# EternityJune25/ComoRAG

Hardware: NVIDIA H100
Metric: queries/sec (higher is better)
Workload: dtype bf16

## Files before the change

comorag_b200/_native.py:

```python
from __future__ import annotations

import ctypes as C
import threading
from pathlib import Path

LIB_PATH = Path(__file__).resolve().parent / "lib" / "libcomorag_b200.so"

CRAG_OK = 0


class NativeError(RuntimeError):
    """A libcomorag_b200 entry point returned a non-zero status."""


_c_i64p = C.POINTER(C.c_int64)
_c_f32p = C.POINTER(C.c_float)

SIGNATURES = {
    "crag_version": (C.c_int, []),
    "crag_last_error": (C.c_char_p, []),
    "crag_sm_count": (C.c_int, []),
    "crag_vmem_reserve": (C.c_int, [C.c_size_t, C.POINTER(C.c_uint64), C.POINTER(C.c_size_t)]),
    "crag_vmem_grow": (C.c_int, [C.c_uint64, C.c_size_t, C.c_size_t]),
    "crag_vmem_release": (C.c_int, [C.c_uint64, C.c_size_t, C.c_size_t]),
    "crag_search_workspace_bytes": (C.c_size_t, [C.c_int, C.c_int]),
    "crag_search_topk": (C.c_int, [C.c_void_p, C.c_int64, C.c_int, C.c_int64, C.c_int64, C.c_void_p, C.c_int,
                                   C.c_int, C.c_void_p, C.c_void_p, C.c_void_p, C.c_void_p, C.c_size_t,
                                   C.c_void_p]),
    "crag_gemm_bf16": (C.c_int, [C.c_void_p, C.c_int64, C.c_void_p, C.c_int64, C.c_void_p, C.c_void_p, C.c_int64,
                                 C.c_void_p, C.c_int64, C.c_int, C.c_int, C.c_int, C.c_int, C.c_void_p]),
    "crag_pool_normalize": (C.c_int, [C.c_void_p, C.c_void_p, C.c_int, C.c_int, C.c_int, C.c_void_p, C.c_void_p,
                                      C.c_int64, C.c_void_p]),
    "crag_encoder_workspace_bytes": (C.c_size_t, None),
    "crag_encoder_forward": (C.c_int, None),
    "crag_encoder_classify": (C.c_int, None),
    "crag_attention_varlen": (C.c_int, [C.c_void_p, C.c_void_p, C.c_int, C.c_int, C.c_int, C.c_int, C.c_void_p,
                                        C.c_void_p]),
    "crag_attention_varlen_tc": (C.c_int, [C.c_void_p, C.c_void_p, C.c_int, C.c_int, C.c_int, C.c_int, C.c_int,
                                           C.c_void_p, C.c_void_p]),
    "crag_layernorm": (C.c_int, [C.c_void_p, C.c_int, C.c_int, C.c_void_p, C.c_void_p, C.c_float, C.c_void_p,
                                 C.c_void_p]),
    "crag_search_topk_after": (C.c_int, [C.c_void_p, C.c_int64, C.c_int, C.c_int64, C.c_int64, C.c_void_p, C.c_int,
                                         C.c_int, C.c_void_p, C.c_void_p, C.c_void_p, C.c_void_p, C.c_void_p,
                                         C.c_void_p, C.c_size_t, C.c_void_p]),
    "crag_search_scan": (C.c_int, [C.c_void_p, C.c_int64, C.c_int, C.c_int64, C.c_void_p, C.c_int, C.c_int, C.c_void_p,
                                   C.c_size_t, C.c_void_p]),
    "crag_search_finalize": (C.c_int, [C.c_void_p, C.c_size_t, C.c_int64, C.c_int, C.c_int, C.c_int64, C.c_void_p,
                                       C.c_void_p, C.c_void_p, C.c_void_p]),
    "crag_merge_topk_packed": (C.c_int, [C.c_void_p, C.c_int64, C.c_int, C.c_int, C.c_int, C.c_void_p, C.c_void_p,
                                         C.c_void_p, C.c_void_p]),
    "crag_ivf_workspace_bytes": (C.c_size_t, [C.c_int, C.c_int64, C.c_int]),
    "crag_ivf_search": (C.c_int, [C.c_void_p, C.c_int64, C.c_int, C.c_int64, C.c_void_p, C.c_void_p, C.c_int, C.c_int64,
                                  C.c_void_p, C.c_void_p, C.c_int, C.c_void_p, C.c_void_p, C.c_int, C.c_int, C.c_void_p,
                                  C.c_void_p, C.c_void_p, C.c_void_p, C.c_size_t, C.c_void_p]),
    "crag_exchange_buffer_bytes": (C.c_size_t, [C.c_int]),
    "crag_search_finalize_exchange": (C.c_int, [C.c_void_p, C.c_size_t, C.c_int64, C.c_int, C.c_int, C.c_int64, C.c_void_p,
                                                C.c_int, C.c_int, C.c_void_p, C.c_void_p, C.c_void_p, C.c_void_p,
                                                C.c_void_p, C.c_void_p]),
    "crag_ivf_assign": (C.c_int, [C.c_void_p, C.c_int64, C.c_int, C.c_int64, C.c_void_p, C.c_int, C.c_void_p, C.c_void_p,
                                  C.c_void_p, C.c_size_t, C.c_void_p]),
    "crag_search_scores": (C.c_int, [C.c_void_p, C.c_int64, C.c_int, C.c_int64, C.c_void_p, C.c_int, C.c_void_p, C.c_int64,
                                     C.c_void_p, C.c_void_p, C.c_size_t, C.c_void_p]),
    "crag_rank_workspace_bytes": (C.c_size_t, [C.c_int64]),
# ... 65 lines not shown
```

comorag_b200/csrc/gemm.cu:

```cuda
#include <cstdlib>

#include "common.cuh"
#include "gemm.cuh"
#include "ptx.cuh"

namespace crag {

constexpr int kGemmBM = 128;
constexpr int kGemmBN = 128;
constexpr int kGemmBK = 64;
constexpr int kGemmConsumerWarps = 8;
constexpr int kGemmThreads = 32 * kGemmConsumerWarps + 32;
constexpr int kGemmStages = 3;

struct GemmLayout {
  static constexpr int kABytes = kGemmBM * kGemmBK * 2;
  static constexpr int kBBytes = kGemmBN * kGemmBK * 2;
  static constexpr int kStageBytes = kABytes + kBBytes;
  static constexpr size_t smem_bytes() { return 1024 + size_t(kGemmStages) * kStageBytes + 2 * kGemmStages * 8; }
};

__device__ __forceinline__ float gelu_erf(float x) {
  const float z = x * 0.70710678118654752f;
  const float az = fabsf(z);
  float t;
  asm("rcp.approx.ftz.f32 %0, %1;" : "=f"(t) : "f"(fmaf(0.3275911f, az, 1.0f)));
  float p = fmaf(1.061405429f, t, -1.453152027f);
  p = fmaf(p, t, 1.421413741f);
  p = fmaf(p, t, -0.284496736f);
  p = fmaf(p, t, 0.254829592f);
  p *= t;
  float e;
  asm("ex2.approx.ftz.f32 %0, %1;" : "=f"(e) : "f"(az * az * -1.4426950408889634f));
  const float erf_abs = fmaf(-p, e, 1.0f);
  const float half_x = 0.5f * x;
  return fmaf(half_x, copysignf(erf_abs, z), half_x);
}

__device__ __forceinline__ uint32_t pack_bf16x2(float a, float b) {
  __nv_bfloat162 v = __floats2bfloat162_rn(a, b);
  return *reinterpret_cast<uint32_t*>(&v);
}

template <int EPI>
__global__ void __launch_bounds__(kGemmThreads, 2)
gemm_bf16_kernel(const __grid_constant__ CUtensorMap tm_a, const __grid_constant__ CUtensorMap tm_b, int M, int N,
                 int K, const float* __restrict__ bias, const __nv_bfloat16* __restrict__ residual, int64_t ldr,
                 __nv_bfloat16* __restrict__ out, int64_t ldo) {
  using L = GemmLayout;
  constexpr int STAGES = kGemmStages;
  extern __shared__ uint8_t smem_raw[];
  uint8_t* smem = reinterpret_cast<uint8_t*>((reinterpret_cast<uintptr_t>(smem_raw) + 1023) & ~uintptr_t(1023));
  uint64_t* bar_full = reinterpret_cast<uint64_t*>(smem + STAGES * L::kStageBytes);
  uint64_t* bar_empty = bar_full + STAGES;

  const int warp = threadIdx.x >> 5;
  const int lane = threadIdx.x & 31;
  int n_blk = blockIdx.x, m_blk = blockIdx.y;
  if constexpr (EPI == GEMM_EPI_SCORES_F32) {
    const int m_blocks = (M + kGemmBM - 1) / kGemmBM;
    m_blk = int(blockIdx.x % unsigned(m_blocks));
    n_blk = int(blockIdx.x / unsigned(m_blocks));
  }
  const int num_kb = (K + kGemmBK - 1) / kGemmBK;

  if (threadIdx.x == 0) {
    for (int s = 0; s < STAGES; ++s) {
      mbar_init(&bar_full[s], 1);
      mbar_init(&bar_empty[s], kGemmConsumerWarps);
    }
    fence_mbar_init();
  }
  __syncthreads();

  if (warp == kGemmConsumerWarps) {
    if (lane == 0) {
      tma_prefetch_desc(&tm_a);
      tma_prefetch_desc(&tm_b);
      const uint64_t pol_w = policy_evict_last();
      int stage = 0;
      uint32_t phase = 0;
      for (int kb = 0; kb < num_kb; ++kb) {
        mbar_wait(&bar_empty[stage], phase ^ 1);
        uint8_t* sa = smem + stage * L::kStageBytes;
        mbar_arrive_expect_tx(&bar_full[stage], L::kStageBytes);
        tma_load_2d(&tm_a, &bar_full[stage], sa, kb * kGemmBK, m_blk * kGemmBM);
        tma_load_2d_hint(&tm_b, &bar_full[stage], sa + L::kABytes, kb * kGemmBK, n_blk * kGemmBN, pol_w);
        if (++stage == STAGES) { stage = 0; phase ^= 1; }
      }
    }
    return;
  }

  const int wg = warp >> 2;
  float acc[kGemmBN / 2];
#pragma unroll
  for (int i = 0; i < kGemmBN / 2; ++i) acc[i] = 0.f;
  int stage = 0, prev = 0;
  uint32_t phase = 0;
  for (int kb = 0; kb < num_kb; ++kb) {
    mbar_wait(&bar_full[stage], phase);
    const uint32_t a_addr = smem_u32(smem + stage * L::kStageBytes) + wg * 64 * 128;
    const uint32_t b_addr = smem_u32(smem + stage * L::kStageBytes + L::kABytes);
    wgmma_fence();
#pragma unroll
    for (int ks = 0; ks < kGemmBK / 16; ++ks)
      wgmma_m64n128k16_ss(acc, wgmma_desc_sw128(a_addr + ks * 32), wgmma_desc_sw128(b_addr + ks * 32), 1u);
    wgmma_commit();
    wgmma_wait<1>();
    if (kb > 0 && lane == 0) mbar_arrive(&bar_empty[prev]);
    prev = stage;
    if (++stage == STAGES) { stage = 0; phase ^= 1; }
  }
  wgmma_wait<0>();
  wgmma_fence_regs(acc);

  if constexpr (EPI == GEMM_EPI_SCORES_F32) {
    float* outf = reinterpret_cast<float*>(out);
    const int srow0 = m_blk * kGemmBM + wg * 64 + (warp & 3) * 16 + (lane >> 2);
    const int scol0 = n_blk * kGemmBN + 2 * (lane & 3);
#pragma unroll
    for (int j = 0; j < kGemmBN / 8; ++j) {
      const int col = scol0 + 8 * j;
#pragma unroll
      for (int h = 0; h < 2; ++h) {
        const int row = srow0 + 8 * h;
        if (row >= M) continue;
        float* p = outf + int64_t(row) * ldo + col;
        if (col + 1 < N) *reinterpret_cast<float2*>(p) = make_float2(acc[4 * j + 2 * h], acc[4 * j + 2 * h + 1]);
        else if (col < N) p[0] = acc[4 * j + 2 * h];
      }
    }
    return;
  }

  const int row0 = m_blk * kGemmBM + wg * 64 + (warp & 3) * 16 + (lane >> 2);
  const int col0 = n_blk * kGemmBN + 2 * (lane & 3);
#pragma unroll
  for (int j = 0; j < kGemmBN / 8; ++j) {
    const int col = col0 + 8 * j;
    if (col >= N) continue;
    const float2 b = __ldg(reinterpret_cast<const float2*>(bias + col));
#pragma unroll
    for (int h = 0; h < 2; ++h) {
      const int row = row0 + 8 * h;
      if (row >= M) continue;
      float x0 = acc[4 * j + 2 * h] + b.x, x1 = acc[4 * j + 2 * h + 1] + b.y;
      if (EPI == GEMM_EPI_BIAS_GELU) {
        x0 = gelu_erf(x0);
        x1 = gelu_erf(x1);
      }
      if (EPI == GEMM_EPI_BIAS_RESIDUAL) {
        const __nv_bfloat162 r = *reinterpret_cast<const __nv_bfloat162*>(residual + int64_t(row) * ldr + col);
        x0 += __bfloat162float(r.x);
        x1 += __bfloat162float(r.y);
      }
      *reinterpret_cast<uint32_t*>(out + int64_t(row) * ldo + col) = pack_bf16x2(x0, x1);
    }
  }
}

template <int EPI>
static int launch_gemm_t(const CUtensorMap& tm_a, const CUtensorMap& tm_b, int M, int N, int K, const float* bias,
                         const __nv_bfloat16* residual, int64_t ldr, __nv_bfloat16* out, int64_t ldo,
                         cudaStream_t stream) {
  auto kern = gemm_bf16_kernel<EPI>;
  {
    static bool done[64] = {false};
    int dev = 0;
    CRAG_CUDA_OK(cudaGetDevice(&dev));
    if (dev < 0 || dev >= 64 || !done[dev]) {
      CRAG_CUDA_OK(cudaFuncSetAttribute(kern, cudaFuncAttributeMaxDynamicSharedMemorySize, int(GemmLayout::smem_bytes())));
      if (dev >= 0 && dev < 64) done[dev] = true;
    }
  }
  const unsigned n_blocks = (N + kGemmBN - 1) / kGemmBN, m_blocks = (M + kGemmBM - 1) / kGemmBM;
  const dim3 grid = EPI == GEMM_EPI_SCORES_F32 ? dim3(m_blocks * n_blocks) : dim3(n_blocks, m_blocks);
  kern<<<grid, kGemmThreads, GemmLayout::smem_bytes(), stream>>>(tm_a, tm_b, M, N, K, bias, residual, ldr, out, ldo);
  CRAG_CUDA_OK(cudaGetLastError());
  return CRAG_OK;
}

int gemm_bf16(const void* a, int64_t lda, const void* w, int64_t ldw, const float* bias, const void* residual,
              int64_t ldr, void* out, int64_t ldo, int M, int N, int K, int epi, cudaStream_t stream) {
  if (M <= 0) return CRAG_OK;
  if (N < 8 || K < 8 || N % 8 != 0 || K % 8 != 0) return fail(CRAG_ERR_INVALID, "gemm: N and K must be positive multiples of 8 (N=%d K=%d)", N, K);
  if (lda % 8 || ldw % 8 || ldo % 8 || (epi == GEMM_EPI_BIAS_RESIDUAL && ldr % 8)) return fail(CRAG_ERR_INVALID, "gemm: leading dimensions must be multiples of 8 elements");
  if (!a || !w || !bias || !out || (epi == GEMM_EPI_BIAS_RESIDUAL && !residual)) return fail(CRAG_ERR_INVALID, "gemm: null pointer");
  if ((uintptr_t(a) | uintptr_t(w) | uintptr_t(out) | uintptr_t(bias) | uintptr_t(residual)) & 15) return fail(CRAG_ERR_INVALID, "gemm: pointers must be 16-byte aligned");
  if ((M + kGemmBM - 1) / kGemmBM > 65535) return fail(CRAG_ERR_INVALID, "gemm: M too large (%d)", M);
  const __nv_bfloat16* res = static_cast<const __nv_bfloat16*>(residual);
  __nv_bfloat16* o = static_cast<__nv_bfloat16*>(out);
  CUtensorMap tm_a, tm_b;
  int rc = make_tmap_bf16_2d(&tm_a, a, uint64_t(M), uint64_t(K), uint64_t(lda) * 2, kGemmBM);
  if (rc != CRAG_OK) return rc;
  rc = make_tmap_bf16_2d(&tm_b, w, uint64_t(N), uint64_t(K), uint64_t(ldw) * 2, kGemmBN);
  if (rc != CRAG_OK) return rc;
  switch (epi) {
    case GEMM_EPI_BIAS: return launch_gemm_t<GEMM_EPI_BIAS>(tm_a, tm_b, M, N, K, bias, res, ldr, o, ldo, stream);
    case GEMM_EPI_BIAS_GELU: return launch_gemm_t<GEMM_EPI_BIAS_GELU>(tm_a, tm_b, M, N, K, bias, res, ldr, o, ldo, stream);
    case GEMM_EPI_BIAS_RESIDUAL: return launch_gemm_t<GEMM_EPI_BIAS_RESIDUAL>(tm_a, tm_b, M, N, K, bias, res, ldr, o, ldo, stream);
  }
  return fail(CRAG_ERR_INVALID, "gemm: unknown epilogue %d", epi);
}

int gemm_scores_f32(const void* a, int64_t lda, const void* w, int64_t ldw, float* out, int64_t ldo, int M, int N,
                    int K, cudaStream_t stream) {
  if (M <= 0 || N <= 0) return CRAG_OK;
  if (K < 64 || K % 64 != 0 || lda % 8 || ldw % 8 || ldo % 2) return fail(CRAG_ERR_INVALID, "gemm scores: K must be a multiple of 64, lda/ldw multiples of 8 and ldo even");
  if ((uintptr_t(a) | uintptr_t(w)) & 15 || uintptr_t(out) & 7) return fail(CRAG_ERR_INVALID, "gemm scores: misaligned pointer");
  if (int64_t((M + kGemmBM - 1) / kGemmBM) * ((N + kGemmBN - 1) / kGemmBN) > int64_t(0x7FFFFFFF)) return fail(CRAG_ERR_INVALID, "gemm scores: too many tiles (M=%d N=%d)", M, N);
  CUtensorMap tm_a, tm_b;
  int rc = make_tmap_bf16_2d(&tm_a, a, uint64_t(M), uint64_t(K), uint64_t(lda) * 2, kGemmBM);
  if (rc != CRAG_OK) return rc;
  rc = make_tmap_bf16_2d(&tm_b, w, uint64_t(N), uint64_t(K), uint64_t(ldw) * 2, kGemmBN);
  if (rc != CRAG_OK) return rc;
  return launch_gemm_t<GEMM_EPI_SCORES_F32>(tm_a, tm_b, M, N, K, nullptr, nullptr, 0, reinterpret_cast<__nv_bfloat16*>(out),
                                            ldo, stream);
}

}

extern "C" int crag_gemm_bf16(const void* a, int64_t lda, const void* w, int64_t ldw, const float* bias,
                              const void* residual, int64_t ldr, void* out, int64_t ldo, int m, int n, int k,
                              int epilogue, crag_stream_t stream) {
  return crag::gemm_bf16(a, lda, w, ldw, bias, residual, ldr, out, ldo, m, n, k, epilogue,
                         static_cast<cudaStream_t>(stream));
}
```

comorag_b200/csrc/gemm.cuh:

```cuda
#pragma once
#include <cuda_runtime.h>
#include <stdint.h>

#include "../../include/comorag_b200.h"

namespace crag {

enum : int {
  GEMM_EPI_BIAS = CRAG_GEMM_BIAS,
  GEMM_EPI_BIAS_GELU = CRAG_GEMM_BIAS_GELU,
  GEMM_EPI_BIAS_RESIDUAL = CRAG_GEMM_BIAS_RESIDUAL,
  GEMM_EPI_SCORES_F32 = 3,
};

int gemm_bf16(const void* a, int64_t lda, const void* w, int64_t ldw, const float* bias, const void* residual,
              int64_t ldr, void* out, int64_t ldo, int M, int N, int K, int epi, cudaStream_t stream);

int gemm_scores_f32(const void* a, int64_t lda, const void* w, int64_t ldw, float* out, int64_t ldo, int M, int N,
                    int K, cudaStream_t stream);

}
```

include/comorag_b200.h:

```cpp
#ifndef COMORAG_B200_H_
#define COMORAG_B200_H_

#include <stddef.h>
#include <stdint.h>

#ifdef __cplusplus
extern "C" {
#endif

#if defined(__GNUC__)
#define CRAG_API __attribute__((visibility("default")))
#else
#define CRAG_API
#endif

#define CRAG_OK 0
#define CRAG_ERR_INVALID (-1)
#define CRAG_ERR_CUDA (-2)
#define CRAG_ERR_WORKSPACE (-3)
#define CRAG_ERR_UNSUPPORTED (-4)

typedef void* crag_stream_t;

CRAG_API int crag_version(void);
// ... 43 lines not shown
                                    int64_t* out_ids, float* out_scores, float* out_minmax, crag_stream_t stream);

CRAG_API size_t crag_exchange_buffer_bytes(int world);
CRAG_API int crag_search_finalize_exchange(const void* workspace, size_t workspace_bytes, int64_t n_rows, int nq, int k,
                                           int64_t row_offset, const uint64_t* peer_bufs, int rank, int world,
                                           uint64_t* epochs, int* status, int64_t* out_ids, float* out_scores,
                                           float* out_minmax, crag_stream_t stream);

CRAG_API int crag_search_scores(const void* corpus, int64_t n_rows, int dim, int64_t corpus_row_stride,
                                const void* queries, int nq, float* out_scores, int64_t out_ld, float* out_minmax,
                                void* workspace, size_t workspace_bytes, crag_stream_t stream);

CRAG_API size_t crag_rank_workspace_bytes(int64_t n);
CRAG_API int crag_rank_scores(const float* scores, int64_t n, int64_t* out_ids, float* out_scores, void* workspace,
                              size_t workspace_bytes, crag_stream_t stream);

CRAG_API size_t crag_ppr_workspace_bytes(int64_t n_vertices, int64_t nnz);
CRAG_API int crag_ppr(const int64_t* row_ptr, const int32_t* col, const float* coef, int64_t n_vertices, int64_t nnz,
                      const float* reset, float damping, int iterations, const int32_t* out_vertices, int64_t n_out,
                      float* out, void* workspace, size_t workspace_bytes, crag_stream_t stream);

CRAG_API size_t crag_ppr_batch_workspace_bytes(int64_t n_vertices, int64_t nnz, int batch);
CRAG_API int crag_ppr_batch(const int64_t* row_ptr, const int32_t* col, const float* coef, int64_t n_vertices,
                            int64_t nnz, const float* resets, int batch, float damping, int iterations,
                            const int32_t* out_vertices, int64_t n_out, float* out, void* workspace,
                            size_t workspace_bytes, crag_stream_t stream);

#define CRAG_GEMM_BIAS 0
#define CRAG_GEMM_BIAS_GELU 1
#define CRAG_GEMM_BIAS_RESIDUAL 2
CRAG_API int crag_gemm_bf16(const void* a, int64_t lda, const void* w, int64_t ldw, const float* bias,
                            const void* residual, int64_t ldr, void* out, int64_t ldo, int m, int n, int k,
                            int epilogue, crag_stream_t stream);

CRAG_API size_t crag_ivf_workspace_bytes(int nlist, int64_t total_tiles, int k);
CRAG_API int crag_ivf_search(const void* residuals, int64_t n_rows_padded, int dim, int64_t row_stride,
                             const int32_t* list_tile_start, const int32_t* list_rows, int nlist,
                             int64_t total_tiles, const int64_t* row_ids, const void* queries, int nq,
                             const int64_t* probed_ids, const float* probed_scores, int nprobe, int k,
                             int64_t* out_ids, float* out_scores, float* out_minmax, void* workspace,
                             size_t workspace_bytes, crag_stream_t stream);

CRAG_API size_t crag_ivf_i8_workspace_bytes(int nlist, int64_t total_tiles, int n_cand);
CRAG_API int crag_ivf_search_i8(const void* residuals_i8, const float* row_scales, int dim8, int64_t row_stride_i8,
                                const void* residuals_bf16, int dim, int64_t row_stride, int64_t n_rows_padded,
                                const int32_t* list_tile_start, const int32_t* list_rows, int nlist,
                                int64_t total_tiles, const int64_t* row_ids, const void* queries_i8,
                                const float* query_scales, const void* queries_bf16, int nq,
                                const int64_t* probed_ids, const float* probed_scores, int nprobe, int n_cand, int k,
                                int64_t* out_ids, float* out_scores, float* out_minmax, void* workspace,
                                size_t workspace_bytes, crag_stream_t stream);

CRAG_API int crag_ivf_assign(const void* rows, int64_t n_rows, int dim, int64_t row_stride, const void* centroids,
                             int nlist, float* best_score, int32_t* best_id, void* workspace, size_t workspace_bytes,
                             crag_stream_t stream);

typedef struct crag_encoder_layer {
  const void* w_qkv;
  const float* b_qkv;
  const void* w_o;
  const float* b_o;
  const float* ln1_g;
  const float* ln1_b;
  const void* w_ff1;
  const float* b_ff1;
  const void* w_ff2;
// ... 66 lines not shown
```

comorag_b200/csrc/attention_tc.cu:

```cuda
#include <cstdlib>

#include "common.cuh"
#include "encoder.cuh"
#include "ptx.cuh"

namespace crag {

constexpr int kAttBM = 128;
constexpr int kAttBN = 64;
constexpr int kAttDH = 64;
constexpr int kAttThreads = 288;
constexpr int kAttTileBytes = 128 * 64 * 2;
constexpr int kAttKVBytes = kAttBN * 64 * 2;
constexpr size_t kAttSmemBytes = 1024 + kAttTileBytes + 4 * kAttKVBytes + 256;

__device__ __forceinline__ float att_exp2(float x) {
  float y;
  asm("ex2.approx.ftz.f32 %0, %1;" : "=f"(y) : "f"(x));
  return y;
}

__device__ __forceinline__ uint32_t att_pack_bf16x2(float a, float b) {
  __nv_bfloat162 v = __floats2bfloat162_rn(a, b);
  return *reinterpret_cast<uint32_t*>(&v);
}

__global__ void __launch_bounds__(kAttThreads, 1)
attention_tc_kernel(const __grid_constant__ CUtensorMap tm_q, const __grid_constant__ CUtensorMap tm_kv,
                    const int32_t* __restrict__ cu_seqlens, int H, float scale_log2e, __nv_bfloat16* __restrict__ ctx) {
  const int seq = blockIdx.z, head = blockIdx.y;
  const int start = __ldg(cu_seqlens + seq);
  const int L = __ldg(cu_seqlens + seq + 1) - start;
  const int q0 = blockIdx.x * kAttBM;
  if (q0 >= L) return;
  const int n_blk = (L + kAttBN - 1) / kAttBN;

  extern __shared__ uint8_t smem_raw[];
  uint8_t* smem = reinterpret_cast<uint8_t*>((reinterpret_cast<uintptr_t>(smem_raw) + 1023) & ~uintptr_t(1023));
  uint8_t* sQ = smem;
  uint8_t* sK = sQ + kAttTileBytes;
  uint8_t* sV = sK + 2 * kAttKVBytes;
  uint64_t* bar_q = reinterpret_cast<uint64_t*>(sV + 2 * kAttKVBytes);
  uint64_t* bar_k_full = bar_q + 1;
  uint64_t* bar_v_full = bar_k_full + 2;
  uint64_t* bar_kv_empty = bar_v_full + 2;

  const int warp = threadIdx.x >> 5, lane = threadIdx.x & 31;
  if (threadIdx.x == 0) {
    mbar_init(bar_q, 1);
    for (int s = 0; s < 2; ++s) {
      mbar_init(&bar_k_full[s], 1);
      mbar_init(&bar_v_full[s], 1);
      mbar_init(&bar_kv_empty[s], 8);
    }
    fence_mbar_init();
  }
  __syncthreads();

  if (warp == 8) {
    if (lane == 0) {
      tma_prefetch_desc(&tm_q);
      tma_prefetch_desc(&tm_kv);
      mbar_arrive_expect_tx(bar_q, kAttTileBytes);
      tma_load_2d(&tm_q, bar_q, sQ, head * kAttDH, start + q0);
      for (int j = 0; j < n_blk; ++j) {
        const int st = j & 1;
        const uint32_t ph = (j >> 1) & 1;
        mbar_wait(&bar_kv_empty[st], ph ^ 1);
        mbar_arrive_expect_tx(&bar_k_full[st], kAttKVBytes);
        tma_load_2d(&tm_kv, &bar_k_full[st], sK + st * kAttKVBytes, H + head * kAttDH, start + j * kAttBN);
        mbar_arrive_expect_tx(&bar_v_full[st], kAttKVBytes);
        tma_load_2d(&tm_kv, &bar_v_full[st], sV + st * kAttKVBytes, 2 * H + head * kAttDH, start + j * kAttBN);
      }
    }
    return;
  }

  const int wg = warp >> 2;
  const uint32_t q_addr = smem_u32(sQ) + wg * 64 * 128;
  float o[32];
#pragma unroll
  for (int i = 0; i < 32; ++i) o[i] = 0.f;
  float m_run[2] = {-INFINITY, -INFINITY}, l_run[2] = {0.f, 0.f};
  mbar_wait(bar_q, 0);
  for (int j = 0; j < n_blk; ++j) {
    const int st = j & 1;
    const uint32_t ph = (j >> 1) & 1;
    mbar_wait(&bar_k_full[st], ph);
    float s[32];
    const uint32_t k_addr = smem_u32(sK + st * kAttKVBytes);
    wgmma_fence();
#pragma unroll
    for (int ks = 0; ks < kAttDH / 16; ++ks)
      wgmma_m64n64k16_ss(s, wgmma_desc_sw128(q_addr + ks * 32), wgmma_desc_sw128(k_addr + ks * 32), ks > 0 ? 1u : 0u);
    wgmma_commit();
    wgmma_wait<0>();
    wgmma_fence_regs(s);

    const int kbase = j * kAttBN + 2 * (lane & 3);
    if (j * kAttBN + kAttBN > L) {
#pragma unroll
      for (int c = 0; c < 8; ++c)
#pragma unroll
        for (int e = 0; e < 2; ++e)
          if (kbase + 8 * c + e >= L) s[4 * c + e] = s[4 * c + 2 + e] = -INFINITY;
    }
    float alpha[2];
#pragma unroll
    for (int h = 0; h < 2; ++h) {
      float mx = -INFINITY;
#pragma unroll
      for (int c = 0; c < 8; ++c) mx = fmaxf(mx, fmaxf(s[4 * c + 2 * h], s[4 * c + 2 * h + 1]));
      mx = fmaxf(mx, __shfl_xor_sync(0xffffffffu, mx, 1));
      mx = fmaxf(mx, __shfl_xor_sync(0xffffffffu, mx, 2));
      const float m_new = fmaxf(m_run[h], mx * scale_log2e);
      alpha[h] = att_exp2(m_run[h] - m_new);
      m_run[h] = m_new;
    }
    uint32_t pa[4][4];
    float rs[2] = {0.f, 0.f};
#pragma unroll
    for (int c = 0; c < 8; ++c) {
#pragma unroll
      for (int h = 0; h < 2; ++h) {
        const float p0 = att_exp2(fmaf(s[4 * c + 2 * h], scale_log2e, -m_run[h]));
        const float p1 = att_exp2(fmaf(s[4 * c + 2 * h + 1], scale_log2e, -m_run[h]));
        rs[h] += p0 + p1;
        pa[c >> 1][(c & 1) * 2 + h] = att_pack_bf16x2(p0, p1);
      }
    }
#pragma unroll
    for (int h = 0; h < 2; ++h) l_run[h] = l_run[h] * alpha[h] + rs[h];
#pragma unroll
    for (int c = 0; c < 8; ++c) {
      o[4 * c + 0] *= alpha[0];
      o[4 * c + 1] *= alpha[0];
      o[4 * c + 2] *= alpha[1];
      o[4 * c + 3] *= alpha[1];
    }
    mbar_wait(&bar_v_full[st], ph);
    const uint32_t v_addr = smem_u32(sV + st * kAttKVBytes);
    wgmma_fence();
#pragma unroll
    for (int kk = 0; kk < kAttBN / 16; ++kk)
      wgmma_m64n64k16_rs_bmn(o, pa[kk], wgmma_desc_sw128(v_addr + kk * 16 * 128), 1u);
    wgmma_commit();
    wgmma_wait<0>();
    wgmma_fence_regs(o);
    __syncwarp();
    if (lane == 0) mbar_arrive(&bar_kv_empty[st]);
  }

#pragma unroll
  for (int h = 0; h < 2; ++h) {
    float l = l_run[h];
    l += __shfl_xor_sync(0xffffffffu, l, 1);
    l += __shfl_xor_sync(0xffffffffu, l, 2);
    const float inv = 1.f / l;
    const int row = q0 + wg * 64 + (warp & 3) * 16 + (lane >> 2) + 8 * h;
    if (row < L) {
      __nv_bfloat16* dst = ctx + int64_t(start + row) * H + head * kAttDH + 2 * (lane & 3);
#pragma unroll
      for (int c = 0; c < 8; ++c)
        *reinterpret_cast<uint32_t*>(dst + 8 * c) = att_pack_bf16x2(o[4 * c + 2 * h] * inv, o[4 * c + 2 * h + 1] * inv);
    }
  }
}

int launch_attention_tc(const void* qkv, const int32_t* cu_seqlens, int n_seqs, int total_tokens, int max_len, int H,
                        int heads, void* ctx, cudaStream_t stream) {
  if (n_seqs <= 0 || max_len <= 0 || total_tokens <= 0) return CRAG_OK;
  if (H / heads != kAttDH) return fail(CRAG_ERR_UNSUPPORTED, "attention_tc: head dim must be 64");
  CUtensorMap tm_q, tm_kv;
  int rc = make_tmap_bf16_2d(&tm_q, qkv, uint64_t(total_tokens), uint64_t(3) * H, uint64_t(3) * H * 2, kAttBM);
  if (rc != CRAG_OK) return rc;
  rc = make_tmap_bf16_2d(&tm_kv, qkv, uint64_t(total_tokens), uint64_t(3) * H, uint64_t(3) * H * 2, kAttBN);
  if (rc != CRAG_OK) return rc;
  const dim3 grid((max_len + kAttBM - 1) / kAttBM, heads, n_seqs);
  const float scale_log2e = 1.4426950408889634f / sqrtf(float(kAttDH));
  {
    static bool done[64] = {false};
    int dev = 0;
    CRAG_CUDA_OK(cudaGetDevice(&dev));
// ... 13 lines not shown
```

Before: 4609.

## Make bf16 GEMM persistent with grid-stride tiles and shuffled 16-byte stores

Converts the TMA/wgmma GEMM kernel into a persistent kernel. Each CTA walks tiles in a grid-stride loop over a grid capped at 2×SM count, so the producer warp can prefetch the next tile's K-blocks while consumers run the current tile's epilogue. The bf16 epilogue now packs results and uses warp shuffles to form 16-byte row stores in place of 4-byte stores. It also adds a max_ctas entry point and an optional compile-time trace. Costs include per-tile mbarrier bookkeeping and extra shuffles, and the tile order changes, which may affect L2 reuse.

```diff
diff --git a/comorag_b200/_native.py b/comorag_b200/_native.py
--- a/comorag_b200/_native.py
+++ b/comorag_b200/_native.py
@@ -29,6 +29,8 @@
                                    C.c_void_p]),
     "crag_gemm_bf16": (C.c_int, [C.c_void_p, C.c_int64, C.c_void_p, C.c_int64, C.c_void_p, C.c_void_p, C.c_int64,
                                  C.c_void_p, C.c_int64, C.c_int, C.c_int, C.c_int, C.c_int, C.c_void_p]),
+    "crag_gemm_bf16_grid": (C.c_int, [C.c_void_p, C.c_int64, C.c_void_p, C.c_int64, C.c_void_p, C.c_void_p, C.c_int64,
+                                      C.c_void_p, C.c_int64, C.c_int, C.c_int, C.c_int, C.c_int, C.c_int, C.c_void_p]),
     "crag_pool_normalize": (C.c_int, [C.c_void_p, C.c_void_p, C.c_int, C.c_int, C.c_int, C.c_void_p, C.c_void_p,
                                       C.c_int64, C.c_void_p]),
     "crag_encoder_workspace_bytes": (C.c_size_t, None),
diff --git a/comorag_b200/csrc/gemm.cu b/comorag_b200/csrc/gemm.cu
--- a/comorag_b200/csrc/gemm.cu
+++ b/comorag_b200/csrc/gemm.cu
@@ -42,6 +42,38 @@
   return *reinterpret_cast<uint32_t*>(&v);
 }
 
+#ifdef CRAG_GEMM_TRACE
+__device__ unsigned long long* g_gemm_trace;
+__device__ unsigned int g_gemm_trace_cap;
+__device__ unsigned int g_gemm_trace_len;
+__device__ __forceinline__ void gemm_trace(uint32_t kind, uint32_t tile) {
+  if (threadIdx.x != 0) return;
+  const unsigned int i = atomicAdd(&g_gemm_trace_len, 1u);
+  if (i >= g_gemm_trace_cap) return;
+  unsigned long long t;
+  uint32_t sm;
+  asm volatile("mov.u64 %0, %%globaltimer;" : "=l"(t));
+  asm volatile("mov.u32 %0, %%smid;" : "=r"(sm));
+  g_gemm_trace[3 * i] = t;
+  g_gemm_trace[3 * i + 1] = (uint64_t(sm) << 32) | kind;
+  g_gemm_trace[3 * i + 2] = (uint64_t(blockIdx.x) << 32) | tile;
+}
+#define GEMM_TRACE(kind, tile) gemm_trace(kind, tile)
+#else
+#define GEMM_TRACE(kind, tile) ((void)0)
+#endif
+
+template <int EPI>
+__device__ __forceinline__ void gemm_tile_coords(uint32_t t, uint32_t m_blocks, uint32_t n_blocks, int& m_blk, int& n_blk) {
+  if constexpr (EPI == GEMM_EPI_SCORES_F32) {
+    m_blk = int(t % m_blocks);
+    n_blk = int(t / m_blocks);
+  } else {
+    n_blk = int(t % n_blocks);
+    m_blk = int(t / n_blocks);
+  }
+}
+
 template <int EPI>
 __global__ void __launch_bounds__(kGemmThreads, 2)
 gemm_bf16_kernel(const __grid_constant__ CUtensorMap tm_a, const __grid_constant__ CUtensorMap tm_b, int M, int N,
@@ -56,12 +88,8 @@
 
   const int warp = threadIdx.x >> 5;
   const int lane = threadIdx.x & 31;
-  int n_blk = blockIdx.x, m_blk = blockIdx.y;
-  if constexpr (EPI == GEMM_EPI_SCORES_F32) {
-    const int m_blocks = (M + kGemmBM - 1) / kGemmBM;
-    m_blk = int(blockIdx.x % unsigned(m_blocks));
-    n_blk = int(blockIdx.x / unsigned(m_blocks));
-  }
+  const uint32_t m_blocks = (M + kGemmBM - 1) / kGemmBM, n_blocks = (N + kGemmBN - 1) / kGemmBN;
+  const uint32_t n_tiles = m_blocks * n_blocks;
   const int num_kb = (K + kGemmBK - 1) / kGemmBK;
 
   if (threadIdx.x == 0) {
@@ -72,97 +100,131 @@
     fence_mbar_init();
   }
   __syncthreads();
-
+  GEMM_TRACE(0, 0);
+
+  int stage = 0;
+  uint32_t phase = 0;
   if (warp == kGemmConsumerWarps) {
     if (lane == 0) {
       tma_prefetch_desc(&tm_a);
       tma_prefetch_desc(&tm_b);
       const uint64_t pol_w = policy_evict_last();
-      int stage = 0;
-      uint32_t phase = 0;
-      for (int kb = 0; kb < num_kb; ++kb) {
-        mbar_wait(&bar_empty[stage], phase ^ 1);
-        uint8_t* sa = smem + stage * L::kStageBytes;
-        mbar_arrive_expect_tx(&bar_full[stage], L::kStageBytes);
-        tma_load_2d(&tm_a, &bar_full[stage], sa, kb * kGemmBK, m_blk * kGemmBM);
-        tma_load_2d_hint(&tm_b, &bar_full[stage], sa + L::kABytes, kb * kGemmBK, n_blk * kGemmBN, pol_w);
-        if (++stage == STAGES) { stage = 0; phase ^= 1; }
+      for (uint32_t t = blockIdx.x; t < n_tiles; t += gridDim.x) {
+        int m_blk, n_blk;
+        gemm_tile_coords<EPI>(t, m_blocks, n_blocks, m_blk, n_blk);
+        for (int kb = 0; kb < num_kb; ++kb) {
+          mbar_wait(&bar_empty[stage], phase ^ 1);
+          uint8_t* sa = smem + stage * L::kStageBytes;
+          mbar_arrive_expect_tx(&bar_full[stage], L::kStageBytes);
+          tma_load_2d(&tm_a, &bar_full[stage], sa, kb * kGemmBK, m_blk * kGemmBM);
+          tma_load_2d_hint(&tm_b, &bar_full[stage], sa + L::kABytes, kb * kGemmBK, n_blk * kGemmBN, pol_w);
+          if (++stage == STAGES) { stage = 0; phase ^= 1; }
+        }
       }
     }
     return;
   }
 
   const int wg = warp >> 2;
-  float acc[kGemmBN / 2];
-#pragma unroll
-  for (int i = 0; i < kGemmBN / 2; ++i) acc[i] = 0.f;
-  int stage = 0, prev = 0;
-  uint32_t phase = 0;
-  for (int kb = 0; kb < num_kb; ++kb) {
-    mbar_wait(&bar_full[stage], phase);
-    const uint32_t a_addr = smem_u32(smem + stage * L::kStageBytes) + wg * 64 * 128;
-    const uint32_t b_addr = smem_u32(smem + stage * L::kStageBytes + L::kABytes);
-    wgmma_fence();
-#pragma unroll
-    for (int ks = 0; ks < kGemmBK / 16; ++ks)
-      wgmma_m64n128k16_ss(acc, wgmma_desc_sw128(a_addr + ks * 32), wgmma_desc_sw128(b_addr + ks * 32), 1u);
-    wgmma_commit();
-    wgmma_wait<1>();
-    if (kb > 0 && lane == 0) mbar_arrive(&bar_empty[prev]);
-    prev = stage;
-    if (++stage == STAGES) { stage = 0; phase ^= 1; }
-  }
-  wgmma_wait<0>();
-  wgmma_fence_regs(acc);
-
-  if constexpr (EPI == GEMM_EPI_SCORES_F32) {
-    float* outf = reinterpret_cast<float*>(out);
-    const int srow0 = m_blk * kGemmBM + wg * 64 + (warp & 3) * 16 + (lane >> 2);
-    const int scol0 = n_blk * kGemmBN + 2 * (lane & 3);
-#pragma unroll
-    for (int j = 0; j < kGemmBN / 8; ++j) {
-      const int col = scol0 + 8 * j;
-#pragma unroll
-      for (int h = 0; h < 2; ++h) {
-        const int row = srow0 + 8 * h;
-        if (row >= M) continue;
-        float* p = outf + int64_t(row) * ldo + col;
-        if (col + 1 < N) *reinterpret_cast<float2*>(p) = make_float2(acc[4 * j + 2 * h], acc[4 * j + 2 * h + 1]);
-        else if (col < N) p[0] = acc[4 * j + 2 * h];
+  for (uint32_t t = blockIdx.x; t < n_tiles; t += gridDim.x) {
+    int m_blk, n_blk;
+    gemm_tile_coords<EPI>(t, m_blocks, n_blocks, m_blk, n_blk);
+    float acc[kGemmBN / 2];
+#pragma unroll
+    for (int i = 0; i < kGemmBN / 2; ++i) acc[i] = 0.f;
+    int prev = 0;
+    for (int kb = 0; kb < num_kb; ++kb) {
+      mbar_wait(&bar_full[stage], phase);
+      if (kb == 0) GEMM_TRACE(1, t);
+      const uint32_t a_addr = smem_u32(smem + stage * L::kStageBytes) + wg * 64 * 128;
+      const uint32_t b_addr = smem_u32(smem + stage * L::kStageBytes + L::kABytes);
+      wgmma_fence();
+#pragma unroll
+      for (int ks = 0; ks < kGemmBK / 16; ++ks)
+        wgmma_m64n128k16_ss(acc, wgmma_desc_sw128(a_addr + ks * 32), wgmma_desc_sw128(b_addr + ks * 32), 1u);
+      wgmma_commit();
+      wgmma_wait<1>();
+      if (kb > 0 && lane == 0) mbar_arrive(&bar_empty[prev]);
+      prev = stage;
+      if (++stage == STAGES) { stage = 0; phase ^= 1; }
+    }
+    wgmma_wait<0>();
+    wgmma_fence_regs(acc);
+    if (lane == 0) mbar_arrive(&bar_empty[prev]);
+    GEMM_TRACE(2, t);
+
+    if constexpr (EPI == GEMM_EPI_SCORES_F32) {
+      float* outf = reinterpret_cast<float*>(out);
+      const int srow0 = m_blk * kGemmBM + wg * 64 + (warp & 3) * 16 + (lane >> 2);
+      const int scol0 = n_blk * kGemmBN + 2 * (lane & 3);
+#pragma unroll
+      for (int j = 0; j < kGemmBN / 8; ++j) {
+        const int col = scol0 + 8 * j;
+#pragma unroll
+        for (int h = 0; h < 2; ++h) {
+          const int row = srow0 + 8 * h;
+          if (row >= M) continue;
+          float* p = outf + int64_t(row) * ldo + col;
+          if (col + 1 < N) *reinterpret_cast<float2*>(p) = make_float2(acc[4 * j + 2 * h], acc[4 * j + 2 * h + 1]);
+          else if (col < N) p[0] = acc[4 * j + 2 * h];
+        }
       }
-    }
-    return;
-  }
-
-  const int row0 = m_blk * kGemmBM + wg * 64 + (warp & 3) * 16 + (lane >> 2);
-  const int col0 = n_blk * kGemmBN + 2 * (lane & 3);
-#pragma unroll
-  for (int j = 0; j < kGemmBN / 8; ++j) {
-    const int col = col0 + 8 * j;
-    if (col >= N) continue;
-    const float2 b = __ldg(reinterpret_cast<const float2*>(bias + col));
-#pragma unroll
-    for (int h = 0; h < 2; ++h) {
-      const int row = row0 + 8 * h;
-      if (row >= M) continue;
-      float x0 = acc[4 * j + 2 * h] + b.x, x1 = acc[4 * j + 2 * h + 1] + b.y;
-      if (EPI == GEMM_EPI_BIAS_GELU) {
-        x0 = gelu_erf(x0);
-        x1 = gelu_erf(x1);
+    } else {
+      const int row0 = m_blk * kGemmBM + wg * 64 + (warp & 3) * 16 + (lane >> 2);
+      const int q = lane & 3;
+#pragma unroll
+      for (int jg = 0; jg < kGemmBN / 32; ++jg) {
+        if (n_blk * kGemmBN + 32 * jg >= N) continue;
+        uint32_t w[2][4];
+#pragma unroll
+        for (int i = 0; i < 4; ++i) {
+          const int j = 4 * jg + i;
+          const int col = n_blk * kGemmBN + 8 * j + 2 * q;
+          const bool col_ok = n_blk * kGemmBN + 8 * j < N;
+          const float2 b = col_ok ? __ldg(reinterpret_cast<const float2*>(bias + col)) : make_float2(0.f, 0.f);
+#pragma unroll
+          for (int h = 0; h < 2; ++h) {
+            const int row = row0 + 8 * h;
+            float x0 = acc[4 * j + 2 * h] + b.x, x1 = acc[4 * j + 2 * h + 1] + b.y;
+            if (EPI == GEMM_EPI_BIAS_GELU) {
+              x0 = gelu_erf(x0);
+              x1 = gelu_erf(x1);
+            }
+            if (EPI == GEMM_EPI_BIAS_RESIDUAL && col_ok && row < M) {
+              const __nv_bfloat162 r = *reinterpret_cast<const __nv_bfloat162*>(residual + int64_t(row) * ldr + col);
+              x0 += __bfloat162float(r.x);
+              x1 += __bfloat162float(r.y);
+            }
+            w[h][i] = pack_bf16x2(x0, x1);
+          }
+        }
+#pragma unroll
+        for (int h = 0; h < 2; ++h) {
+          uint32_t* v = w[h];
+#pragma unroll
+          for (int i = 0; i < 2; ++i) {
+            const uint32_t r = __shfl_xor_sync(0xffffffffu, (q & 2) ? v[i] : v[i + 2], 2);
+            if (q & 2) v[i] = r; else v[i + 2] = r;
+          }
+#pragma unroll
+          for (int i = 0; i < 4; i += 2) {
+            const uint32_t r = __shfl_xor_sync(0xffffffffu, (q & 1) ? v[i] : v[i + 1], 1);
+            if (q & 1) v[i] = r; else v[i + 1] = r;
+          }
+          const int row = row0 + 8 * h;
+          const int col = n_blk * kGemmBN + 8 * (4 * jg + q);
+          if (row < M && col < N)
+            *reinterpret_cast<uint4*>(out + int64_t(row) * ldo + col) = make_uint4(v[0], v[1], v[2], v[3]);
+        }
       }
-      if (EPI == GEMM_EPI_BIAS_RESIDUAL) {
-        const __nv_bfloat162 r = *reinterpret_cast<const __nv_bfloat162*>(residual + int64_t(row) * ldr + col);
-        x0 += __bfloat162float(r.x);
-        x1 += __bfloat162float(r.y);
-      }
-      *reinterpret_cast<uint32_t*>(out + int64_t(row) * ldo + col) = pack_bf16x2(x0, x1);
-    }
+    }
+    GEMM_TRACE(3, t);
   }
 }
 
 template <int EPI>
 static int launch_gemm_t(const CUtensorMap& tm_a, const CUtensorMap& tm_b, int M, int N, int K, const float* bias,
-                         const __nv_bfloat16* residual, int64_t ldr, __nv_bfloat16* out, int64_t ldo,
+                         const __nv_bfloat16* residual, int64_t ldr, __nv_bfloat16* out, int64_t ldo, int max_ctas,
                          cudaStream_t stream) {
   auto kern = gemm_bf16_kernel<EPI>;
   {
@@ -174,21 +236,28 @@
       if (dev >= 0 && dev < 64) done[dev] = true;
     }
   }
-  const unsigned n_blocks = (N + kGemmBN - 1) / kGemmBN, m_blocks = (M + kGemmBM - 1) / kGemmBM;
-  const dim3 grid = EPI == GEMM_EPI_SCORES_F32 ? dim3(m_blocks * n_blocks) : dim3(n_blocks, m_blocks);
+  const int64_t n_tiles = int64_t((M + kGemmBM - 1) / kGemmBM) * ((N + kGemmBN - 1) / kGemmBN);
+  if (max_ctas == 0) {
+    const int sms = sm_count();
+    if (sms < 0) return CRAG_ERR_CUDA;
+    max_ctas = 2 * sms;
+  }
+  const unsigned grid = unsigned(n_tiles < max_ctas ? n_tiles : max_ctas);
   kern<<<grid, kGemmThreads, GemmLayout::smem_bytes(), stream>>>(tm_a, tm_b, M, N, K, bias, residual, ldr, out, ldo);
   CRAG_CUDA_OK(cudaGetLastError());
   return CRAG_OK;
 }
 
 int gemm_bf16(const void* a, int64_t lda, const void* w, int64_t ldw, const float* bias, const void* residual,
-              int64_t ldr, void* out, int64_t ldo, int M, int N, int K, int epi, cudaStream_t stream) {
+              int64_t ldr, void* out, int64_t ldo, int M, int N, int K, int epi, cudaStream_t stream, int max_ctas) {
   if (M <= 0) return CRAG_OK;
   if (N < 8 || K < 8 || N % 8 != 0 || K % 8 != 0) return fail(CRAG_ERR_INVALID, "gemm: N and K must be positive multiples of 8 (N=%d K=%d)", N, K);
   if (lda % 8 || ldw % 8 || ldo % 8 || (epi == GEMM_EPI_BIAS_RESIDUAL && ldr % 8)) return fail(CRAG_ERR_INVALID, "gemm: leading dimensions must be multiples of 8 elements");
   if (!a || !w || !bias || !out || (epi == GEMM_EPI_BIAS_RESIDUAL && !residual)) return fail(CRAG_ERR_INVALID, "gemm: null pointer");
   if ((uintptr_t(a) | uintptr_t(w) | uintptr_t(out) | uintptr_t(bias) | uintptr_t(residual)) & 15) return fail(CRAG_ERR_INVALID, "gemm: pointers must be 16-byte aligned");
   if ((M + kGemmBM - 1) / kGemmBM > 65535) return fail(CRAG_ERR_INVALID, "gemm: M too large (%d)", M);
+  if (int64_t((M + kGemmBM - 1) / kGemmBM) * ((N + kGemmBN - 1) / kGemmBN) > int64_t(0x7FFFFFFF)) return fail(CRAG_ERR_INVALID, "gemm: too many tiles (M=%d N=%d)", M, N);
+  if (max_ctas < 0) return fail(CRAG_ERR_INVALID, "gemm: max_ctas must be >= 0 (%d)", max_ctas);
   const __nv_bfloat16* res = static_cast<const __nv_bfloat16*>(residual);
   __nv_bfloat16* o = static_cast<__nv_bfloat16*>(out);
   CUtensorMap tm_a, tm_b;
@@ -197,9 +266,9 @@
   rc = make_tmap_bf16_2d(&tm_b, w, uint64_t(N), uint64_t(K), uint64_t(ldw) * 2, kGemmBN);
   if (rc != CRAG_OK) return rc;
   switch (epi) {
-    case GEMM_EPI_BIAS: return launch_gemm_t<GEMM_EPI_BIAS>(tm_a, tm_b, M, N, K, bias, res, ldr, o, ldo, stream);
-    case GEMM_EPI_BIAS_GELU: return launch_gemm_t<GEMM_EPI_BIAS_GELU>(tm_a, tm_b, M, N, K, bias, res, ldr, o, ldo, stream);
-    case GEMM_EPI_BIAS_RESIDUAL: return launch_gemm_t<GEMM_EPI_BIAS_RESIDUAL>(tm_a, tm_b, M, N, K, bias, res, ldr, o, ldo, stream);
+    case GEMM_EPI_BIAS: return launch_gemm_t<GEMM_EPI_BIAS>(tm_a, tm_b, M, N, K, bias, res, ldr, o, ldo, max_ctas, stream);
+    case GEMM_EPI_BIAS_GELU: return launch_gemm_t<GEMM_EPI_BIAS_GELU>(tm_a, tm_b, M, N, K, bias, res, ldr, o, ldo, max_ctas, stream);
+    case GEMM_EPI_BIAS_RESIDUAL: return launch_gemm_t<GEMM_EPI_BIAS_RESIDUAL>(tm_a, tm_b, M, N, K, bias, res, ldr, o, ldo, max_ctas, stream);
   }
   return fail(CRAG_ERR_INVALID, "gemm: unknown epilogue %d", epi);
 }
@@ -216,7 +285,7 @@
   rc = make_tmap_bf16_2d(&tm_b, w, uint64_t(N), uint64_t(K), uint64_t(ldw) * 2, kGemmBN);
   if (rc != CRAG_OK) return rc;
   return launch_gemm_t<GEMM_EPI_SCORES_F32>(tm_a, tm_b, M, N, K, nullptr, nullptr, 0, reinterpret_cast<__nv_bfloat16*>(out),
-                                            ldo, stream);
+                                            ldo, 0, stream);
 }
 
 }
@@ -227,3 +296,23 @@
   return crag::gemm_bf16(a, lda, w, ldw, bias, residual, ldr, out, ldo, m, n, k, epilogue,
                          static_cast<cudaStream_t>(stream));
 }
+
+extern "C" int crag_gemm_bf16_grid(const void* a, int64_t lda, const void* w, int64_t ldw, const float* bias,
+                                   const void* residual, int64_t ldr, void* out, int64_t ldo, int m, int n, int k,
+                                   int epilogue, int max_ctas, crag_stream_t stream) {
+  return crag::gemm_bf16(a, lda, w, ldw, bias, residual, ldr, out, ldo, m, n, k, epilogue,
+                         static_cast<cudaStream_t>(stream), max_ctas);
+}
+
+#ifdef CRAG_GEMM_TRACE
+extern "C" CRAG_API int64_t crag_gemm_trace_reset(void* buf, int64_t cap) {
+  unsigned int len = 0, zero = 0, c = unsigned(cap);
+  unsigned long long* p = static_cast<unsigned long long*>(buf);
+  if (cudaDeviceSynchronize() != cudaSuccess || cudaMemcpyFromSymbol(&len, crag::g_gemm_trace_len, sizeof len) != cudaSuccess ||
+      cudaMemcpyToSymbol(crag::g_gemm_trace, &p, sizeof p) != cudaSuccess ||
+      cudaMemcpyToSymbol(crag::g_gemm_trace_cap, &c, sizeof c) != cudaSuccess ||
+      cudaMemcpyToSymbol(crag::g_gemm_trace_len, &zero, sizeof zero) != cudaSuccess)
+    return -1;
+  return len;
+}
+#endif
diff --git a/comorag_b200/csrc/gemm.cuh b/comorag_b200/csrc/gemm.cuh
--- a/comorag_b200/csrc/gemm.cuh
+++ b/comorag_b200/csrc/gemm.cuh
@@ -14,7 +14,8 @@
 };
 
 int gemm_bf16(const void* a, int64_t lda, const void* w, int64_t ldw, const float* bias, const void* residual,
-              int64_t ldr, void* out, int64_t ldo, int M, int N, int K, int epi, cudaStream_t stream);
+              int64_t ldr, void* out, int64_t ldo, int M, int N, int K, int epi, cudaStream_t stream,
+              int max_ctas = 0);
 
 int gemm_scores_f32(const void* a, int64_t lda, const void* w, int64_t ldw, float* out, int64_t ldo, int M, int N,
                     int K, cudaStream_t stream);
diff --git a/include/comorag_b200.h b/include/comorag_b200.h
--- a/include/comorag_b200.h
+++ b/include/comorag_b200.h
@@ -99,6 +99,9 @@
 CRAG_API int crag_gemm_bf16(const void* a, int64_t lda, const void* w, int64_t ldw, const float* bias,
                             const void* residual, int64_t ldr, void* out, int64_t ldo, int m, int n, int k,
                             int epilogue, crag_stream_t stream);
+CRAG_API int crag_gemm_bf16_grid(const void* a, int64_t lda, const void* w, int64_t ldw, const float* bias,
+                                 const void* residual, int64_t ldr, void* out, int64_t ldo, int m, int n, int k,
+                                 int epilogue, int max_ctas, crag_stream_t stream);
 
 CRAG_API size_t crag_ivf_workspace_bytes(int nlist, int64_t total_tiles, int k);
 CRAG_API int crag_ivf_search(const void* residuals, int64_t n_rows_padded, int dim, int64_t row_stride,
```

Result: no change. 4596 (median of 6 runs) (-0.3%).

## Software-pipeline QK and PV wgmma, drop producer warp, deepen KV ring

Applied to the files above, without the earlier changes.

Restructures the attention main loop so the QK^T wgmma for block j is issued together with the PV wgmma for block j-1, and softmax of j runs while PV is still in flight. This aims to hide tensor-core latency behind the exp/max work. The dedicated TMA producer warp is removed: thread 0 prefills four KV stages and refills each slot after its consumers release it. The KV ring grows from two to four stages and launch bounds now request two CTAs per SM. In exchange, thread 0 stalls on the empty barrier during refills, and register pressure from the double P buffers may conflict with the two-CTA occupancy target.

```diff
diff --git a/comorag_b200/csrc/attention_tc.cu b/comorag_b200/csrc/attention_tc.cu
--- a/comorag_b200/csrc/attention_tc.cu
+++ b/comorag_b200/csrc/attention_tc.cu
@@ -9,10 +9,11 @@
 constexpr int kAttBM = 128;
 constexpr int kAttBN = 64;
 constexpr int kAttDH = 64;
-constexpr int kAttThreads = 288;
+constexpr int kAttStages = 4;
+constexpr int kAttThreads = 256;
 constexpr int kAttTileBytes = 128 * 64 * 2;
 constexpr int kAttKVBytes = kAttBN * 64 * 2;
-constexpr size_t kAttSmemBytes = 1024 + kAttTileBytes + 4 * kAttKVBytes + 256;
+constexpr size_t kAttSmemBytes = 1024 + kAttTileBytes + 2 * kAttStages * kAttKVBytes + 256;
 
 __device__ __forceinline__ float att_exp2(float x) {
   float y;
@@ -25,7 +26,55 @@
   return *reinterpret_cast<uint32_t*>(&v);
 }
 
-__global__ void __launch_bounds__(kAttThreads, 1)
+__device__ __forceinline__ void att_issue_qk(float (&s)[32], uint32_t q_addr, uint32_t k_addr) {
+#pragma unroll
+  for (int ks = 0; ks < kAttDH / 16; ++ks)
+    wgmma_m64n64k16_ss(s, wgmma_desc_sw128(q_addr + ks * 32), wgmma_desc_sw128(k_addr + ks * 32), ks > 0 ? 1u : 0u);
+}
+
+__device__ __forceinline__ void att_issue_pv(float (&o)[32], const uint32_t (&pa)[4][4], uint32_t v_addr) {
+#pragma unroll
+  for (int kk = 0; kk < kAttBN / 16; ++kk) wgmma_m64n64k16_rs_bmn(o, pa[kk], wgmma_desc_sw128(v_addr + kk * 16 * 128), 1u);
+}
+
+__device__ __forceinline__ void att_softmax(float (&s)[32], int key0, int L, int lane, float scale_log2e,
+                                            float (&m_run)[2], float (&l_run)[2], float (&alpha)[2],
+                                            uint32_t (&pa)[4][4]) {
+  const int kbase = key0 + 2 * (lane & 3);
+  if (key0 + kAttBN > L) {
+#pragma unroll
+    for (int c = 0; c < 8; ++c)
+#pragma unroll
+      for (int e = 0; e < 2; ++e)
+        if (kbase + 8 * c + e >= L) s[4 * c + e] = s[4 * c + 2 + e] = -INFINITY;
+  }
+#pragma unroll
+  for (int h = 0; h < 2; ++h) {
+    float mx = -INFINITY;
+#pragma unroll
+    for (int c = 0; c < 8; ++c) mx = fmaxf(mx, fmaxf(s[4 * c + 2 * h], s[4 * c + 2 * h + 1]));
+    mx = fmaxf(mx, __shfl_xor_sync(0xffffffffu, mx, 1));
+    mx = fmaxf(mx, __shfl_xor_sync(0xffffffffu, mx, 2));
+    const float m_new = fmaxf(m_run[h], mx * scale_log2e);
+    alpha[h] = att_exp2(m_run[h] - m_new);
+    m_run[h] = m_new;
+  }
+  float rs[2] = {0.f, 0.f};
+#pragma unroll
+  for (int c = 0; c < 8; ++c) {
+#pragma unroll
+    for (int h = 0; h < 2; ++h) {
+      const float p0 = att_exp2(fmaf(s[4 * c + 2 * h], scale_log2e, -m_run[h]));
+      const float p1 = att_exp2(fmaf(s[4 * c + 2 * h + 1], scale_log2e, -m_run[h]));
+      rs[h] += p0 + p1;
+      pa[c >> 1][(c & 1) * 2 + h] = att_pack_bf16x2(p0, p1);
+    }
+  }
+#pragma unroll
+  for (int h = 0; h < 2; ++h) l_run[h] = l_run[h] * alpha[h] + rs[h];
+}
+
+__global__ void __launch_bounds__(kAttThreads, 2)
 attention_tc_kernel(const __grid_constant__ CUtensorMap tm_q, const __grid_constant__ CUtensorMap tm_kv,
                     const int32_t* __restrict__ cu_seqlens, int H, float scale_log2e, __nv_bfloat16* __restrict__ ctx) {
   const int seq = blockIdx.z, head = blockIdx.y;
@@ -39,16 +88,16 @@
   uint8_t* smem = reinterpret_cast<uint8_t*>((reinterpret_cast<uintptr_t>(smem_raw) + 1023) & ~uintptr_t(1023));
   uint8_t* sQ = smem;
   uint8_t* sK = sQ + kAttTileBytes;
-  uint8_t* sV = sK + 2 * kAttKVBytes;
-  uint64_t* bar_q = reinterpret_cast<uint64_t*>(sV + 2 * kAttKVBytes);
+  uint8_t* sV = sK + kAttStages * kAttKVBytes;
+  uint64_t* bar_q = reinterpret_cast<uint64_t*>(sV + kAttStages * kAttKVBytes);
   uint64_t* bar_k_full = bar_q + 1;
-  uint64_t* bar_v_full = bar_k_full + 2;
-  uint64_t* bar_kv_empty = bar_v_full + 2;
+  uint64_t* bar_v_full = bar_k_full + kAttStages;
+  uint64_t* bar_kv_empty = bar_v_full + kAttStages;
 
   const int warp = threadIdx.x >> 5, lane = threadIdx.x & 31;
   if (threadIdx.x == 0) {
     mbar_init(bar_q, 1);
-    for (int s = 0; s < 2; ++s) {
+    for (int s = 0; s < kAttStages; ++s) {
       mbar_init(&bar_k_full[s], 1);
       mbar_init(&bar_v_full[s], 1);
       mbar_init(&bar_kv_empty[s], 8);
@@ -57,23 +106,25 @@
   }
   __syncthreads();
 
-  if (warp == 8) {
-    if (lane == 0) {
-      tma_prefetch_desc(&tm_q);
-      tma_prefetch_desc(&tm_kv);
-      mbar_arrive_expect_tx(bar_q, kAttTileBytes);
-      tma_load_2d(&tm_q, bar_q, sQ, head * kAttDH, start + q0);
-      for (int j = 0; j < n_blk; ++j) {
-        const int st = j & 1;
-        const uint32_t ph = (j >> 1) & 1;
-        mbar_wait(&bar_kv_empty[st], ph ^ 1);
-        mbar_arrive_expect_tx(&bar_k_full[st], kAttKVBytes);
-        tma_load_2d(&tm_kv, &bar_k_full[st], sK + st * kAttKVBytes, H + head * kAttDH, start + j * kAttBN);
-        mbar_arrive_expect_tx(&bar_v_full[st], kAttKVBytes);
-        tma_load_2d(&tm_kv, &bar_v_full[st], sV + st * kAttKVBytes, 2 * H + head * kAttDH, start + j * kAttBN);
-      }
-    }
-    return;
+  auto kv_load = [&](int j) {
+    const int st = j % kAttStages;
+    mbar_arrive_expect_tx(&bar_k_full[st], kAttKVBytes);
+    tma_load_2d(&tm_kv, &bar_k_full[st], sK + st * kAttKVBytes, H + head * kAttDH, start + j * kAttBN);
+    mbar_arrive_expect_tx(&bar_v_full[st], kAttKVBytes);
+    tma_load_2d(&tm_kv, &bar_v_full[st], sV + st * kAttKVBytes, 2 * H + head * kAttDH, start + j * kAttBN);
+  };
+  auto refill = [&](int jd) {
+    if (threadIdx.x == 0 && jd + kAttStages < n_blk) {
+      mbar_wait(&bar_kv_empty[jd % kAttStages], (jd / kAttStages) & 1);
+      kv_load(jd + kAttStages);
+    }
+  };
+  if (threadIdx.x == 0) {
+    tma_prefetch_desc(&tm_q);
+    tma_prefetch_desc(&tm_kv);
+    mbar_arrive_expect_tx(bar_q, kAttTileBytes);
+    tma_load_2d(&tm_q, bar_q, sQ, head * kAttDH, start + q0);
+    for (int j = 0; j < n_blk && j < kAttStages; ++j) kv_load(j);
   }
 
   const int wg = warp >> 2;
@@ -81,56 +132,36 @@
   float o[32];
 #pragma unroll
   for (int i = 0; i < 32; ++i) o[i] = 0.f;
-  float m_run[2] = {-INFINITY, -INFINITY}, l_run[2] = {0.f, 0.f};
+  float m_run[2] = {-INFINITY, -INFINITY}, l_run[2] = {0.f, 0.f}, alpha[2];
+  float s[32];
+  uint32_t pa0[4][4], pa1[4][4];
   mbar_wait(bar_q, 0);
-  for (int j = 0; j < n_blk; ++j) {
-    const int st = j & 1;
-    const uint32_t ph = (j >> 1) & 1;
-    mbar_wait(&bar_k_full[st], ph);
-    float s[32];
-    const uint32_t k_addr = smem_u32(sK + st * kAttKVBytes);
+
+  mbar_wait(&bar_k_full[0], 0);
+  wgmma_fence();
+  att_issue_qk(s, q_addr, smem_u32(sK));
+  wgmma_commit();
+  wgmma_wait<0>();
+  wgmma_fence_regs(s);
+  att_softmax(s, 0, L, lane, scale_log2e, m_run, l_run, alpha, pa0);
+
+  auto step = [&](int j, const uint32_t (&p_prev)[4][4], uint32_t (&p_next)[4][4]) {
+    const int st = j % kAttStages, stp = (j - 1) % kAttStages;
+    mbar_wait(&bar_k_full[st], (j / kAttStages) & 1);
+    mbar_wait(&bar_v_full[stp], ((j - 1) / kAttStages) & 1);
     wgmma_fence();
-#pragma unroll
-    for (int ks = 0; ks < kAttDH / 16; ++ks)
-      wgmma_m64n64k16_ss(s, wgmma_desc_sw128(q_addr + ks * 32), wgmma_desc_sw128(k_addr + ks * 32), ks > 0 ? 1u : 0u);
+    att_issue_qk(s, q_addr, smem_u32(sK + st * kAttKVBytes));
     wgmma_commit();
+    att_issue_pv(o, p_prev, smem_u32(sV + stp * kAttKVBytes));
+    wgmma_commit();
+    wgmma_wait<1>();
+    wgmma_fence_regs(s);
+    att_softmax(s, j * kAttBN, L, lane, scale_log2e, m_run, l_run, alpha, p_next);
     wgmma_wait<0>();
-    wgmma_fence_regs(s);
-
-    const int kbase = j * kAttBN + 2 * (lane & 3);
-    if (j * kAttBN + kAttBN > L) {
-#pragma unroll
-      for (int c = 0; c < 8; ++c)
-#pragma unroll
-        for (int e = 0; e < 2; ++e)
-          if (kbase + 8 * c + e >= L) s[4 * c + e] = s[4 * c + 2 + e] = -INFINITY;
-    }
-    float alpha[2];
-#pragma unroll
-    for (int h = 0; h < 2; ++h) {
-      float mx = -INFINITY;
-#pragma unroll
-      for (int c = 0; c < 8; ++c) mx = fmaxf(mx, fmaxf(s[4 * c + 2 * h], s[4 * c + 2 * h + 1]));
-      mx = fmaxf(mx, __shfl_xor_sync(0xffffffffu, mx, 1));
-      mx = fmaxf(mx, __shfl_xor_sync(0xffffffffu, mx, 2));
-      const float m_new = fmaxf(m_run[h], mx * scale_log2e);
-      alpha[h] = att_exp2(m_run[h] - m_new);
-      m_run[h] = m_new;
-    }
-    uint32_t pa[4][4];
-    float rs[2] = {0.f, 0.f};
-#pragma unroll
-    for (int c = 0; c < 8; ++c) {
-#pragma unroll
-      for (int h = 0; h < 2; ++h) {
-        const float p0 = att_exp2(fmaf(s[4 * c + 2 * h], scale_log2e, -m_run[h]));
-        const float p1 = att_exp2(fmaf(s[4 * c + 2 * h + 1], scale_log2e, -m_run[h]));
-        rs[h] += p0 + p1;
-        pa[c >> 1][(c & 1) * 2 + h] = att_pack_bf16x2(p0, p1);
-      }
-    }
-#pragma unroll
-    for (int h = 0; h < 2; ++h) l_run[h] = l_run[h] * alpha[h] + rs[h];
+    wgmma_fence_regs(o);
+    __syncwarp();
+    if (lane == 0) mbar_arrive(&bar_kv_empty[stp]);
+    refill(j - 1);
 #pragma unroll
     for (int c = 0; c < 8; ++c) {
       o[4 * c + 0] *= alpha[0];
@@ -138,17 +169,26 @@
       o[4 * c + 2] *= alpha[1];
       o[4 * c + 3] *= alpha[1];
     }
-    mbar_wait(&bar_v_full[st], ph);
-    const uint32_t v_addr = smem_u32(sV + st * kAttKVBytes);
+  };
+  auto drain = [&](const uint32_t (&p_last)[4][4]) {
+    const int stp = (n_blk - 1) % kAttStages;
+    mbar_wait(&bar_v_full[stp], ((n_blk - 1) / kAttStages) & 1);
     wgmma_fence();
-#pragma unroll
-    for (int kk = 0; kk < kAttBN / 16; ++kk)
-      wgmma_m64n64k16_rs_bmn(o, pa[kk], wgmma_desc_sw128(v_addr + kk * 16 * 128), 1u);
+    att_issue_pv(o, p_last, smem_u32(sV + stp * kAttKVBytes));
     wgmma_commit();
     wgmma_wait<0>();
     wgmma_fence_regs(o);
-    __syncwarp();
-    if (lane == 0) mbar_arrive(&bar_kv_empty[st]);
+  };
+  int j = 1;
+  for (; j + 1 < n_blk; j += 2) {
+    step(j, pa0, pa1);
+    step(j + 1, pa1, pa0);
+  }
+  if (j < n_blk) {
+    step(j, pa0, pa1);
+    drain(pa1);
+  } else {
+    drain(pa0);
   }
 
 #pragma unroll
```

Result: no change. 4604 before, 4609 after, median of 6 (+0.1%).
